# wild-firefox/FreeRL

Measured on AMD Instinct MI355X. Metric: learner_updates_per_sec, higher is better.
Workload: dtype f32; 1 GPU; TD3.learn() (BASELINE configs[1] algorithm; north_star synthetic shape): obs_dim 8, act_dim 2, batch 256, replay 1e6 rows filled, hidden 128, policy_freq 2, device-drawn indices/noise; learners_per_gpu=512, kernel_family=chained (one eight-wave workgroup per learner, two waves per SIMD), rows_per_workgroup=256, lds_bytes=160128, parallelism=seeds sharded over 1 GPU(s), no data-path collective, collective=metric all-reduce: none (single process)

## Files before the change

freerl_amd/csrc/device/chain_net.hpp:

```cpp
#pragma once
#include "chain.hpp"
#include "ppo_timing.hpp"

#if defined(FRL_PPO_TIMING) && defined(FRL_BWD_TIMING)
#define BWD_T0() long long b_prev_ = clock64()
#define BWD_T(i) do { const long long n_ = clock64(); if (threadIdx.x == 0 && blockIdx.x == 0) atomicAdd((unsigned long long*)&g_ppo_clk[1][i], (unsigned long long)(n_ - b_prev_)); b_prev_ = n_; } while (0)
#else
#define BWD_T0() do {} while (0)
#define BWD_T(i) do {} while (0)
#endif
#ifndef FRL_LANES_OPAQUE4
#define FRL_LANES_OPAQUE4 1
#endif
#ifndef FRL_FW_HALF
#define FRL_FW_HALF 1
#endif

namespace frl {

constexpr int kChainBatch = 256;


struct ChainLds {
    lds_f w1, w2, w3, b1, b2, b3, ls, ea, eb, ab, yb, q1, lpn, red, ex;
};
constexpr int chain_lds_floats() { return 8 * 256 + 64 * 256 + 8 * 256 + 2 * 8192 + 128 + 128 + 16 + 16 + kChainBatch * 4 + 3 * kChainBatch + 64; }
constexpr int chain8_lds_floats() { return chain_lds_floats() + 1024; }

template <int NW>
struct HeadGradT {
    static constexpr int OT = kHT / NW;
    f32x4 g2[OT][kHT], g1[OT], g3[OT];
    float gb1[OT], gb2[OT], gb3;
};
using HeadGrad = HeadGradT<4>;

typedef int i32x4_t __attribute__((ext_vector_type(4)));
struct AdamBuf { __amdgpu_buffer_rsrc_t th, mm, vv, tg; };
constexpr int kAdamDrop = 0x40000000;
__device__ __forceinline__ AdamBuf adam_buf(g_f th, g_f mA, g_f vA, g_f tg, int bytes) {
    AdamBuf B;
// ... 17 lines not shown
    return __builtin_nontemporal_load(reinterpret_cast<const FRL_GLB f32x4*>(p));
#else
    return ld4(p);
#endif
}
__device__ __forceinline__ f32x4 buf_ld4(__amdgpu_buffer_rsrc_t r, int voff, int soff) {
    return __builtin_bit_cast(f32x4, __builtin_amdgcn_raw_buffer_load_b128(r, voff, soff, FRL_ADAM_AUX_LD));
}
__device__ __forceinline__ void buf_st4(__amdgpu_buffer_rsrc_t r, int voff, int const_off, const f32x4& v) {
    __builtin_amdgcn_raw_buffer_store_b128(__builtin_bit_cast(i32x4_t, v), r, voff + const_off, 0, FRL_ADAM_AUX_ST);
}



template <int NW>
struct ChainNetT {
    static_assert(NW == 4 || NW == 8, "4 or 8 waves per workgroup");
    static constexpr int OT = kHT / NW, kThreads = 64 * NW, kRows = 16 * NW;
    using Grad = HeadGradT<NW>;
    ChainLds S;
    int tid, l, w, i16, q, fslot, tslot;
    int lane2, lane1;

    __device__ __forceinline__ void init(float* smem) {
        lds_f p = (lds_f)smem;
        S.w1 = p; p += kHT * 256;
        S.w2 = p; p += kHT * kHT * 256;
        S.w3 = p; p += kHT * 256;
        S.ea = p; p += kHT * 4 * 256;
        S.eb = p; p += kHT * 4 * 256;
        S.b1 = p; p += kHid;
        S.b2 = p; p += kHid;
        S.b3 = p; p += 16;
        S.ls = p; p += 16;
        if constexpr (NW == 4) {
            S.ab = p; p += kChainBatch * 4;
            S.yb = p; p += kChainBatch;
            S.q1 = p; p += kChainBatch;
            S.lpn = p; p += kChainBatch;
            S.red = p; p += 64;
            S.ex = S.ab;
        } else {
            S.yb = p; p += kChainBatch;
            S.q1 = p; p += kChainBatch;
            S.lpn = p; p += kChainBatch;
            S.red = p; p += 64;
            S.ab = p; p += kChainBatch * 4;
            S.ex = S.ab;
        }
        init_lanes();
    }
    __device__ __forceinline__ void init_lanes() {
        tid = threadIdx.x; l = tid & 63; w = __builtin_amdgcn_readfirstlane(tid >> 6); i16 = l & 15; q = l >> 4;
        fslot = (q * 16 + (i16 ^ q)) << 2;
        tslot = (((i16 >> 2) * 16) << 2) + (i16 & 3);
        lane2 = 4 * (w * OT * kHT * 256 + fslot);
        lane1 = 4 * (w * OT * 256 + fslot);
    }

    struct LaneK { int i16, q, fslot, tslot; };
    __device__ __forceinline__ LaneK lanes() const {
        int L = l;
        if constexpr (NW == 8 || FRL_LANES_OPAQUE4) asm volatile("" : "+v"(L));
        LaneK K;
        K.i16 = L & 15; K.q = L >> 4;
        K.fslot = (K.q * 16 + (K.i16 ^ K.q)) << 2;
        K.tslot = (((K.i16 >> 2) * 16) << 2) + (K.i16 & 3);
        return K;
    }

    struct StageRegs { f32x4 t2[64 / NW], t1[8 / NW], t3[8 / NW]; float bb1, bb2, bb3, lsv; };
    __device__ __forceinline__ StageRegs stage_fetch(g_cf th, int head, int extra_n = 0) const {
        th += head * kHeadFloats;
        StageRegs R;
#pragma unroll
        for (int j = 0; j < 64 / NW; ++j) R.t2[j] = ld4_stage(th + kL2w + 4 * (tid + kThreads * j));
// ... 484 lines not shown
```

freerl_amd/csrc/engine_plan.hpp:

```cpp
#pragma once
#include <algorithm>
#include <cstdarg>
#include <cstddef>
#include <cstdio>
#include <cstring>
#include <string>
#include <utility>
#include <vector>

#include "../../include/freerl_hip.h"
#include "frl_desc.h"

namespace frl {

inline int pad16(int x) { return (x + 15) / 16 * 16; }
inline int pad32(int x) { return (x + 31) / 32 * 32; }

inline constexpr char kFrlLearn[] = "frl_learn";
struct AlgoTraits {
    const char* name;
    const char* learn;
    const char* act_hint;
    bool index_action;
    bool discrete_head;
// ... 33 lines not shown
constexpr int kLdsDqnFused = dqn2_lds_floats() * (int)sizeof(float);
constexpr int kLdsChain4 = critic2_lds_floats() * (int)sizeof(float), kLdsChain8 = critic8_lds_floats() * (int)sizeof(float);
constexpr int kLdsSolo = std::max(solo_lds_floats(), critic2_lds_floats()) * (int)sizeof(float);
constexpr int kLdsSolow = solow_lds_floats() * (int)sizeof(float);
constexpr int kLdsWide = wide_lds_floats() * (int)sizeof(float), kLdsWide16 = wide16_lds_floats_host() * (int)sizeof(float);
constexpr int kLdsMasac = 160 * 1024;
constexpr int kLdsAtt = 160 * 1024;

struct PlanLimits {
    int n_cus = 256;
    int lds_per_cu = 160 * 1024;
};
struct PlanKnobs {
    int assume_cus = 0;
    int rc = 0;
    int cps = 0;
    bool solow_narrow = false;
    int critic_v2 = -1;
    int solo = -1;
    int solo_maxp = 2 * kSoloMaxP;
    int solow = -1;
    bool solow_helpers = true;
    int chain_waves = 8;
};
inline bool knob_flag(int tri, bool dflt) { return tri < 0 ? dflt : tri != 0; }

struct EngineFacts {
    LearnFamily family = FAM_ROWCHUNK;
    int lds_bytes = 0;
    bool has_nets = false;
    int noisy_per_set = 0;
    size_t idx_count = 0, noise_count = 0;
    size_t alpha_count = 0, steps_count = 0;
    int solo_stride = 0;
    int solow_row_wgs = 0;
    int solow_wgs = 0;
    size_t act_wk_slot = 0;
    int chain_waves = 8;
    int n_cus = 256;
    int lds_per_cu = 160 * 1024;
};
struct EnginePlan : EngineFacts {
    EngineDesc h;
};

__attribute__((format(printf, 2, 3))) inline int plan_refuse(std::string* message, const char* fmt, ...) {
    char buf[512];
    va_list ap;
    va_start(ap, fmt);
    vsnprintf(buf, sizeof buf, fmt, ap);
    va_end(ap);
    if (message) *message = buf;
    return FRL_ERR_INVALID;
}

inline int build_net(NetDesc& N, const std::vector<std::pair<int, int>>& layers_in , int heads,
                     int hidden_act, int out_act, int extra_n, int n_shadow = 0) {
    memset(&N, 0, sizeof N);
    std::vector<std::pair<int, int>> layers = layers_in;
    for (int i = 0; i < n_shadow; ++i) layers.push_back(layers_in.back());
    N.n_layers = (int)layers.size();
// ... 164 lines not shown
}

inline int dqn_split_for(const EngineDesc& h, int batch, int pc, int split_knob) {
    const int nchunks = (batch + 63) / 64;
    int split = (pc <= 16) ? std::min(std::min(4, nchunks), h.S) : 1;
    if (split_knob >= 0) split = std::max(1, std::min(std::min(split_knob, nchunks), h.S));
    return split;
}

inline int family_lds_bytes(LearnFamily fam, int chain_waves) {
    switch (fam) {
        case FAM_DQN_FUSED: return kLdsDqnFused;
        case FAM_CHAINED: return chain_waves == 4 ? kLdsChain4 : kLdsChain8;
        case FAM_SOLO: return kLdsSolo;
        case FAM_SOLOW: return kLdsSolow;
        case FAM_WIDE: return kLdsWide;
        case FAM_WIDE16: return kLdsWide16;
        case FAM_ATT: return kLdsAtt;
        case FAM_MASAC: return kLdsMasac;
        case FAM_ROWCHUNK: break;
    }
    return 0;
}

struct LearnPath { bool chained; int bytes, rows; };
inline LearnPath learn_path(const EngineDesc& h, const EngineFacts& f, LearnFamily fam, int batch, int dqn_split) {
    int bytes = family_lds_bytes(fam, f.chain_waves), rows = batch;
    switch (fam) {
        case FAM_ROWCHUNK: case FAM_ATT: case FAM_MASAC: bytes = f.lds_bytes; rows = h.rc; break;
        case FAM_DQN_FUSED: rows = std::min(((batch + 63) / 64 + dqn_split - 1) / dqn_split * 64, batch); break;
        case FAM_SOLO: bytes = solo_lds_floats() * (int)sizeof(float); rows = 16 * (kSoloWG / h.solo); break;
        case FAM_SOLOW: rows = 16 * (h.solow / std::max(1, f.solow_row_wgs)); break;
        default: break;
    }
    return {fam != FAM_ROWCHUNK && fam != FAM_ATT && fam != FAM_MASAC, bytes, rows};
}

inline int check_create_args(const frl_config& c, const frl_config_ext* ext, std::string* message) {
    int state_dim = 0;
    if (ext) {
        if (ext->size != (int)sizeof(frl_config_ext)) return plan_refuse(message, "frl_config_ext.size %d != sizeof(frl_config_ext) %d", ext->size, (int)sizeof(frl_config_ext));
        if (ext->state_dim < 0) return plan_refuse(message, "frl_config_ext.state_dim %d must be >= 0", ext->state_dim);
        if (ext->state_rows != FRL_STATE_ROWS_POSITION && ext->state_rows != FRL_STATE_ROWS_SAMPLE)
            return plan_refuse(message, "frl_config_ext.state_rows %d (FRL_STATE_ROWS_POSITION or FRL_STATE_ROWS_SAMPLE)", ext->state_rows);
        state_dim = ext->state_dim;
    }
// ... 169 lines not shown
        off += h.net[i].size;
        const int nl = h.net[i].n_layers / h.net[i].heads;
        if (c.algo == FRL_ALGO_MADDPG_ATT && (i & 1)) {
            kin = std::max(kin, h.net[i].L[ATT_E].k_pad);
            continue;
        }
        for (int hd = 0; hd < h.net[i].heads; ++hd) {
            kin = std::max(kin, h.net[i].L[hd * nl].k_pad);
            outp = std::max(outp, h.net[i].L[hd * nl + nl - 1].n_pad);
        }
    }
    h.learner_stride = pad32(off);
    h.lds_kin_pad = kin;
    h.lds_out_pad = outp;
}

inline int plan_sizes(const frl_config& c, const PlanKnobs& knobs, EnginePlan& pl, std::string* message) {
    EngineDesc& h = pl.h;
    const RecordDesc& R = h.rec;
    const AlgoTraits& T = algo_traits(c.algo);
    const int H = h.hidden;
    pl.family = choose_engine_family(pl, knobs);
    pl.chain_waves = knobs.chain_waves == 4 ? 4 : 8;
    h.act_max = 1;
    for (int j = 0; j < c.n_agents; ++j) h.act_max = std::max(h.act_max, R.act_dim[j]);
    h.lds_hbufs = 1;
    for (int i = 0; i < h.n_nets; ++i)
        if (h.net[i].n_layers / std::max(1, h.net[i].heads) > 2) h.lds_hbufs = 2;
    h.lds_batch_pad = 128;
    h.lds_act_pad = (std::max(R.act_total, 1) + 3) / 4 * 4;
    if (h.c51_atoms) h.lds_act_pad = std::max(h.lds_act_pad, (std::max(h.c51_atoms, c.act_dim[0]) + 3) / 4 * 4);
    if (T.vector_reward) h.lds_act_pad = std::max(h.lds_act_pad, (h.reward_dim + 3) / 4 * 4);
    bool one_wg_per_net = false;
    bool whole_cu = false;
    int call_rows = h.batch_max;
    switch (c.algo) {
        case FRL_ALGO_PPO:
            if (c.discrete) h.lds_act_pad = std::max(h.lds_act_pad, pad16(c.act_dim[0]));
            if (c.actor_dist == 1) h.lds_act_pad = std::max(h.lds_act_pad, pad16(2 * c.act_dim[0]));
            one_wg_per_net = true;
            break;
        case FRL_ALGO_SAC_DISCRETE:
            h.lds_act_pad = std::max(h.lds_act_pad, (c.act_dim[0] + 3) / 4 * 4);
            break;
        case FRL_ALGO_GAIL:
            h.lds_act_pad = std::max(h.lds_act_pad, ((H + 31) / 32 + 3) / 4 * 4);
// ... 125 lines not shown
```

freerl_amd/csrc/frl_api.hip:

```cpp
#include <hip/hip_runtime.h>

#include <chrono>
#include <cmath>
#include <cstdarg>
#include <cstdio>
#include <cstdlib>
#include <cstring>
#include <string>
#include <vector>

#include "../../include/freerl_hip.h"
#include "frl_desc.h"
#include "engine_plan.hpp"
#include "host_mem.hpp"

#include "kernels.h"
#ifdef FRL_UNITY
#include "kernels_replay.hip"
#include "kernels_update.hip"
#include "kernels_dqn.hip"
#include "kernels_critic.hip"
#include "kernels_actor.hip"
#include "kernels_act.hip"
#include "kernels_ppo.hip"
// ... 217 lines not shown
    if (e->stream) hipStreamDestroy(e->stream);
    delete e;
    return FRL_OK;
}

static LearnKernels resolve_learn_kernels(LearnFamily fam, int chain_waves, const EngineDesc& h);
static hipError_t set_family_lds_attributes(LearnFamily fam);

extern "C" int frl_create(const frl_config* cfg, frl_engine** out) { return frl_create_ex(cfg, nullptr, out); }

static PlanKnobs create_knobs() {
    auto tri = [](const char* name) { return env_set(name) ? (int)env_flag(name, false) : -1; };
    PlanKnobs k;
    k.assume_cus = env_int("FRL_ASSUME_CUS", k.assume_cus);
    k.rc = env_int("FRL_RC", k.rc);
    k.cps = env_int("FRL_CPS", k.cps);
    k.solow_narrow = env_flag("FRL_SOLOW_NARROW", k.solow_narrow);
    k.critic_v2 = tri("FRL_CRITIC_V2");
    k.solo = tri("FRL_SOLO");
    k.solo_maxp = env_int("FRL_SOLO_MAXP", k.solo_maxp);
    k.solow = tri("FRL_SOLOW");
    k.solow_helpers = env_flag("FRL_SOLOW_HELPERS", k.solow_helpers);
    k.chain_waves = env_int("FRL_CHAIN_WAVES", k.chain_waves);
    return k;
}

extern "C" int frl_create_ex(const frl_config* cfg, const frl_config_ext* ext, frl_engine** out) {
    if (!cfg || !out) return fail(FRL_ERR_INVALID, "cfg/out is NULL");
    *out = nullptr;
    const frl_config& c = *cfg;
    std::string why;
    if (const int rc = check_create_args(c, ext, &why)) return fail(rc, "%s", why.c_str());
    int ndev = 0;
    if (hipGetDeviceCount(&ndev) != hipSuccess || ndev == 0)
        return fail(FRL_ERR_NO_DEVICE, "no HIP device visible: the engine has no CPU fallback");
    if (c.device_id < 0 || c.device_id >= ndev) return fail(FRL_ERR_INVALID, "device_id %d of %d", c.device_id, ndev);
    HIP_TRY(hipSetDevice(c.device_id));
    PlanLimits limits;
    hipDeviceProp_t prop;
    if (hipGetDeviceProperties(&prop, c.device_id) == hipSuccess) {
        limits.n_cus = std::max(1, prop.multiProcessorCount);
        limits.lds_per_cu = (int)std::max<size_t>(prop.maxSharedMemoryPerMultiProcessor, prop.sharedMemPerBlock);
    }
    EnginePlan plan;
    if (const int rc = plan_engine(c, ext, limits, create_knobs(), &plan, &why)) return fail(rc, "%s", why.c_str());

// ... 1010 lines not shown
```

freerl_amd/csrc/frl_api_learn.inc:

```

enum LearnKernelStage { LK_CRITIC, LK_CRITIC_NV, LK_ACTOR, LK_STEP };
struct LearnKernelRow {
    LearnFamily fam;
    int stage;
    int sub;
    int lds_bytes;
    KernelPtr k[2][2];
};
static const LearnKernelRow kLearnKernels[] = {
    {FAM_DQN_FUSED, LK_CRITIC, 0, kLdsDqnFused, {{dqn_fused_kernel, dqn_fused_kernel}, {dqn_fused_kernel, dqn_fused_kernel}}},
    {FAM_CHAINED, LK_CRITIC, 8, kLdsChain8, {{ac_critic_v2_single_kernel, ac_critic_v2_single_kernel}, {ac_critic_v2_twin_kernel, ac_critic_v2_twin_kernel}}},
    {FAM_CHAINED, LK_CRITIC_NV, 8, kLdsChain8, {{ac_critic_v2_single_nv_kernel, ac_critic_v2_single_nv_kernel}, {ac_critic_v2_twin_nv_kernel, ac_critic_v2_twin_nv_kernel}}},
    {FAM_CHAINED, LK_ACTOR, 8, kLdsChain8, {{ac_actor_v2_kernel, ac_actor_v2_kernel}, {ac_actor_v2_kernel, ac_actor_v2_kernel}}},
    {FAM_CHAINED, LK_CRITIC, 4, kLdsChain4, {{ac_critic_v2w4_single_kernel, ac_critic_v2w4_single_kernel}, {ac_critic_v2w4_twin_kernel, ac_critic_v2w4_twin_kernel}}},
    {FAM_CHAINED, LK_ACTOR, 4, kLdsChain4, {{ac_actor_v2w4_kernel, ac_actor_v2w4_kernel}, {ac_actor_v2w4_kernel, ac_actor_v2w4_kernel}}},
    {FAM_SOLO, LK_CRITIC, 16, kLdsSolo, {{solo_critic_single_kernel, solo_critic_single_kernel}, {solo_critic_twin_kernel, solo_critic_twin_kernel}}},
    {FAM_SOLO, LK_ACTOR, 16, kLdsSolo, {{solo_actor_kernel, solo_actor_kernel}, {solo_actor_kernel, solo_actor_kernel}}},
    {FAM_SOLO, LK_CRITIC, 8, kLdsSolo, {{solo_critic_single_w8_kernel, solo_critic_single_w8_kernel}, {solo_critic_twin_w8_kernel, solo_critic_twin_w8_kernel}}},
    {FAM_SOLO, LK_ACTOR, 8, kLdsSolo, {{solo_actor_w8_kernel, solo_actor_w8_kernel}, {solo_actor_w8_kernel, solo_actor_w8_kernel}}},
    {FAM_SOLOW, LK_CRITIC, 1, kLdsSolow, {{solow_critic_h1a1_kernel, solow_critic_h1a2_kernel}, {solow_critic_h2a1_kernel, solow_critic_h2a2_kernel}}},
    {FAM_SOLOW, LK_ACTOR, 1, kLdsSolow, {{solow_actor_a1_kernel, solow_actor_a2_kernel}, {solow_actor_a1_kernel, solow_actor_a2_kernel}}},
    {FAM_SOLOW, LK_STEP, 1, kLdsSolow, {{solow_step_h1a1_kernel, solow_step_h1a2_kernel}, {solow_step_h2a1_kernel, solow_step_h2a2_kernel}}},
    {FAM_SOLOW, LK_CRITIC, 2, kLdsSolow, {{solow_critic_ma_h1a1_kernel, solow_critic_ma_h1a2_kernel}, {solow_critic_ma_h2a1_kernel, solow_critic_ma_h2a2_kernel}}},
    {FAM_SOLOW, LK_ACTOR, 2, kLdsSolow, {{solow_actor_ma_a1_kernel, solow_actor_ma_a2_kernel}, {solow_actor_ma_a1_kernel, solow_actor_ma_a2_kernel}}},
// ... 109 lines not shown
    prof_begin(e, actor ? PK_GRAD_ACTOR : PK_GRAD_CRITIC);
    hipLaunchKernelGGL(k, grid_chunks, dim3(256), e->lds_bytes, s.st, e->d, a, ns);
    prof_end(e);
    AdamArgs ad{};
    ad.ns = ns; ad.batch = a.batch; ad.eps = a.adam_eps; ad.beta1 = a.beta1; ad.beta2 = a.beta2; ad.clip = a.clip_norm;
    ad.tau = a.tau; ad.alpha_lr = a.alpha_lr; ad.target_entropy = a.target_entropy; ad.p0 = s.p0; ad.G = h.Gmax;
    if (actor) {
        ad.which = 1; ad.lr = a.actor_lr; ad.wd = 0.f; ad.soft = maddpg ? 0 : 1; ad.sac_alpha = sac ? 1 : 0;
    } else {
        ad.which = 0; ad.lr = a.critic_lr; ad.wd = a.critic_wd;
        ad.soft = (h.algo == ALGO_DQN) ? 1 : ((!maddpg && a.do_actor) ? 1 : 0);
    }
    prof_begin(e, actor ? PK_ADAM_ACTOR : PK_ADAM_CRITIC);
    launch_adam(e, s.st, ad, s.units, grid_adam);
    prof_end(e);
}

static void launch_chained(frl_engine* e, const LearnStage& s, LearnArgs a) {
    const LearnKernels& K = e->kern;
    LearnKernel k = K.actor.k;
    if (s.stage == 0) {
        a.stagger = env_int("FRL_STAGGER", 0);
        a.stagger_groups = env_int("FRL_STAGGER_GROUPS", 4); a.stagger_wgs = e->n_cus;
        const RecordDesc& R = e->h.rec;
        const bool nv = R.nobs_off[0] % 4 == 0 && R.nobs_off[0] + 16 <= R.stride && R.rew_off % 2 == 0 && R.done_off == R.rew_off + 1 && !env_set("FRL_CRITIC2_NOVEC");
        k = (nv && K.critic_nv.k) ? K.critic_nv.k : K.critic.k;
    }
    prof_begin(e, s.stage == 0 ? PK_GRAD_CRITIC : PK_GRAD_ACTOR);
    hipLaunchKernelGGL(k, dim3(s.pc), dim3(K.block), (size_t)K.lds_bytes, s.st, e->d, a);
    prof_end(e);
}

static void launch_wide(frl_engine* e, const LearnStage& s, const LearnArgs& a) {
    const LearnKernels& K = e->kern;
    prof_begin(e, s.stage == 0 ? PK_GRAD_CRITIC : PK_GRAD_ACTOR);
    hipLaunchKernelGGL(s.stage == 0 ? K.critic.k : K.actor.k, dim3(s.units), dim3(K.block), (size_t)K.lds_bytes, s.st, e->d, a);
    prof_end(e);
}

static SoloArgs solo_args(frl_engine* e) {
    SoloArgs sa{e->d_solo_slab, e->d_solo_part, e->d_solo_bar, e->d_solo_err, e->solo_bar_base, e->solo_stride, nullptr, nullptr, 0ull};
    if (e->h.solow) { sa.tiles = e->h.solow; sa.bar2 = e->d_solow_bar2; sa.row_wgs = e->solow_row_wgs; sa.update_wgs = e->solow_wgs; }
    e->solo_bar_base += kSoloWG;
    return sa;
}

static bool predraw_slots(frl_engine* e, SoloArgs& sa, size_t slot_stride, bool read, bool may_write) {
    if (read) sa.pre_read = e->d_solo_pre + (size_t)(e->solo_pre_seq & 1) * slot_stride;
    if (may_write) {
        sa.pre_write = e->d_solo_pre + (size_t)((e->solo_pre_seq + 1) & 1) * slot_stride;
        sa.pre_counter = e->rng_counter;
    }
// ... 243 lines not shown
```

freerl_amd/csrc/frl_desc.h:

```cpp
#pragma once
#include <stdint.h>

namespace frl {

constexpr int kMaxLayers = 7;
constexpr int kMaxAgents = 8;
constexpr int kMaxNets = 2 * kMaxAgents;

enum Act : int { ACT_NONE = 0, ACT_RELU = 1, ACT_TANH = 2, ACT_LEAKY_RELU = 3 };
constexpr float kLeakySlope = 0.01f;
enum Algo : int { ALGO_DQN = 0, ALGO_DDPG = 1, ALGO_TD3 = 2, ALGO_SAC = 3, ALGO_MADDPG = 4, ALGO_PPO = 5, ALGO_SAC_DISCRETE = 6,
                  ALGO_REINFORCE = 7, ALGO_ENVELOPE_DQN = 8, ALGO_ENVELOPE_DDPG = 9, ALGO_GAIL = 10, ALGO_MAPPO = 11, ALGO_IPPO = 12, ALGO_HAPPO = 13,
                  ALGO_MADDPG_ATT = 14, ALGO_MASAC = 15 };

struct LayerDesc {
    int n, k;
    int n_pad, k_pad;
    int w_off, b_off;
};

struct NetDesc {
    int n_layers;
    int size;
    int n_params;
// ... 145 lines not shown
};

struct LearnArgs {
    int batch;
    int size;
    int device_rng;
    int do_actor;
    float gamma, tau;
    float actor_lr, critic_lr, alpha_lr;
    float adam_eps, beta1, beta2;
    float critic_wd;
    float clip_norm;
    float policy_noise, noise_clip, max_action, policy_noise_scale;
    int use_policy_noise;
    float target_entropy;
    unsigned long long rng_counter;
    int p0, p_count;
    int double_dqn;
    int use_isw;
    int dqn_split;
    int stagger;
    int stagger_groups;
    int stagger_wgs;
    int fuse_actor;
    int huber;
    float huber_delta;
    int agent;
};

}
```

freerl_amd/csrc/kernels_actor2.hip:

```cpp
#include <hip/hip_runtime.h>

#include "kernels.h"
#include "device/chain_net.hpp"
#include "device/ppo_timing.hpp"

namespace frl {

template <int NW, int TA>
__device__ __forceinline__ void ac_actor_v2_body(const EngineDesc& D, const LearnArgs& a, float* smem) {
    constexpr int kRC = 16 * NW, kRowsT = kRC * TA;
    constexpr int kNC = kChainBatch / kRC, kNCT = kChainBatch / kRowsT;
    static_assert(kNCT >= 1, "a chunk of passes A / B is at most the whole batch");
    const int p = a.p0 + blockIdx.x;
    const RecordDesc& R = D.rec;
    const NetDesc& NA = D.net[0];
    const NetDesc& NC = D.net[1];
    using Net = ChainNetT<NW>;
    Net C;
    C.init(smem);
    const ChainLds& S = C.S;
    const int tid = C.tid, l = C.l, w = C.w, i16 = C.i16, q = C.q;
    const int B = a.batch, O = R.obs_dim[0], A = R.act_dim[0];
    const size_t lbase = (size_t)p * D.learner_stride;
    g_f thA = as_global(D.theta + lbase + D.net_off[0]);
    g_f tgA = as_global(D.target + lbase + D.net_off[0]);
    g_f mA = as_global(D.m + lbase + D.net_off[0]);
    g_f vA = as_global(D.v + lbase + D.net_off[0]);
    g_cf thC = as_global(D.theta + lbase + D.net_off[1]);
    g_cf ring = as_global(D.replay + (size_t)p * D.capacity * R.stride);
    g_ci idx = as_global_i(D.idx + (size_t)p * D.batch_max);
    const float invB = 1.f / (float)B;
    const bool sac = (D.algo == ALGO_SAC);
    const float alpha = sac ? D.alpha[p * 4 + 3] : 0.f;
    const int am = D.act_max;
    g_cf noise1 = as_global(D.noise + ((size_t)p * D.noise_sets + 1) * D.batch_max * am);
    const int nq = sac ? NC.heads : 1;
    const float dqv = sac ? -0.5f * invB : -invB;
    const int nchunks = (B + kRC - 1) / kRC, nch2 = (B + kRowsT - 1) / kRowsT;
    lds_f dab = S.eb;

    int ridxT[kNC], ridx[kNC];
#pragma unroll
    for (int j4 = 0; j4 < kNC; ++j4) {
        const int rowT = (j4 / TA) * kRowsT + 16 * TA * w + (j4 % TA) * 16 + i16, row = j4 * kRC + 16 * w + i16;
        ridxT[j4] = rowT < B ? idx[rowT] : -1;
// ... 10 lines not shown
            for (int cc = 1; cc < kNCT; ++cc) ri = c2 == cc ? ridxT[TA * cc + t] : ri;
            if (ri >= 0) {
                g_cf rec = ring + (size_t)ri * R.stride;
#pragma unroll
                for (int e = 0; e < 4; ++e)
                    if (4 * q + e < O) X.x[t][e] = rec[R.obs_off[0] + 4 * q + e];
            }
        }
        return X;
    };
    auto load_obs = [&](int c) {
        f32x4 x = {0.f, 0.f, 0.f, 0.f};
        const int ri = pick(ridx, c);
        if (ri >= 0) {
            g_cf rec = ring + (size_t)ri * R.stride;
#pragma unroll
            for (int e = 0; e < 4; ++e)
                if (4 * q + e < O) x[e] = rec[R.obs_off[0] + 4 * q + e];
        }
        return x;
    };

    float lpsum = 0.f;
    PPO_T0();
    RowIn2 nxt2 = load_obs2(0);
    typename Net::StageRegs pend = C.stage_fetch((g_cf)thA, 0, NA.extra_n);
    C.stage_commit(pend);
    PPO_T(0);
    for (int c2 = 0; c2 < nch2; ++c2) {
        const RowIn2 cur = nxt2;
        nxt2 = load_obs2(c2 + 1 < nch2 ? c2 + 1 : 0);
        if (c2 + 1 == nch2) pend = C.stage_fetch(thC, 0);
        f32x4 z[TA], h1[TA][kHT], h2[TA][kHT];
        C.template forward_vh<TA>(cur.x, h1, h2, z, A);
#pragma unroll
        for (int t = 0; t < TA; ++t) {
            const int row = c2 * kRowsT + 16 * TA * w + 16 * t + i16;
            if (q == 0 && row < kChainBatch) {
                f32x4 an = {0.f, 0.f, 0.f, 0.f};
#pragma unroll
                for (int r = 0; r < 4; ++r) {
                    if (r < A && row < B) {
                        if (sac) {
                            an[r] = sac_sample(z[t][r], S.ls[r], noise1[(size_t)row * am + r], lpsum);
                        } else {
                            an[r] = tanhf(z[t][r]);
                        }
// ... 113 lines not shown
    lds_barrier();
    auto red_sum = [&](int base) {
        float v = S.red[base];
#pragma unroll
        for (int i = 1; i < NW; ++i) v += S.red[base + i];
        return v;
    };
    float g_extra = 0.f, ss_extra = 0.f;
    if (sac) {
#pragma unroll
        for (int r = 0; r < 4; ++r) {
            if (r < A) {
                const float raw = S.ls[r];
                const float gr = log_std_grad_open(raw) ? red_sum(24 + 8 * r) : 0.f;
                ss_extra += gr * gr;
                if (i16 == r) g_extra = gr;
            }
        }
    }
    const float total = sqrtf(red_sum(0) + ss_extra);
    const float qtot = red_sum(8);
    const float lptot = red_sum(16);
    const int t = __float_as_int(S.red[56]) + 1;
    const double bc1 = 1.0 - powi_d((double)a.beta1, t), bc2 = 1.0 - powi_d((double)a.beta2, t);
    AdamCoef co;
    co.coef = a.clip_norm > 0.f ? fminf(a.clip_norm / (total + 1e-6f), 1.f) : 1.f;
    co.step = (float)((double)a.actor_lr / bc1); co.inv_bc2s = 1.f / (float)sqrt(bc2);
    co.w1 = 1.f - a.beta1; co.w2 = 1.f - a.beta2; co.beta2 = a.beta2; co.eps = a.adam_eps; co.wd = 0.f;
    co.tk = 1.f - a.tau; co.tau = a.tau;
    PPO_T(5);
    C.template adam_head<true, 0, true>(g, thA, mA, vA, tgA, co, O, A, g_extra, sac ? NA.extra_n : 0);
    PPO_T(6);
    PPO_TDUMP();
    if (tid == 0) {
        steps[0] = t;
        float* st = D.stats + (size_t)p * ST_COUNT;
        st[ST_ACTOR_LOSS] = actor_loss_stat(sac, qtot, lptot, alpha, invB);
        st[ST_ACTOR_GNORM] = total;
        if (sac) sac_alpha_step(D.alpha + p * 4, st, steps, alpha, -lptot * invB, a.target_entropy, a.beta1, a.beta2, a.alpha_lr);
    }
}

#ifndef FRL_ACTOR8_TA
#define FRL_ACTOR8_TA 1
#endif
__global__ __launch_bounds__(512) void ac_actor_v2_kernel(const EngineDesc* __restrict__ Dp, LearnArgs a) {
    extern __shared__ __attribute__((aligned(16))) float smem[];
    ac_actor_v2_body<8, FRL_ACTOR8_TA>(*Dp, a, smem);
}
__global__ __launch_bounds__(256) void ac_actor_v2w4_kernel(const EngineDesc* __restrict__ Dp, LearnArgs a) {
    extern __shared__ __attribute__((aligned(16))) float smem[];
    ac_actor_v2_body<4, 2>(*Dp, a, smem);
}

}
```

freerl_amd/csrc/kernels_critic2.hip:

```cpp
#include <hip/hip_runtime.h>

#include "kernels.h"
#include "device/chain_net.hpp"
#include "device/ppo_timing.hpp"

#if defined(FRL_BWD_TIMING)
#undef PPO_UDUMP
#define PPO_UDUMP() do {} while (0)
#endif

namespace frl {

#ifndef FRL_CRITIC2_TT
#define FRL_CRITIC2_TT 2
#endif
#ifndef FRL_CRITIC2_AHEAD
#define FRL_CRITIC2_AHEAD 1
#endif
template <bool TWIN, int TT, int NW, bool NVEC>
__device__ __forceinline__ void ac_critic_v2_body(const EngineDesc& D, const LearnArgs& a, float* smem) {
    constexpr int kRC = 16 * NW;
    constexpr int kRowsT = kRC * TT;
    constexpr int kNC = kChainBatch / kRC;
    constexpr int kNCT = kChainBatch / kRowsT;
    static_assert(kNCT >= 1, "a target-pass chunk is at most the whole batch");
    constexpr int NH = TWIN ? 2 : 1;
    const int p = a.p0 + blockIdx.x;
    const RecordDesc& R = D.rec;
    const NetDesc& NA = D.net[0];
    const NetDesc& NC = D.net[1];
    using Net = ChainNetT<NW>;
    Net C;
    C.init(smem);
    const ChainLds& S = C.S;
    const int tid = C.tid, l = C.l, w = C.w, i16 = C.i16, q = C.q;
    const int B = a.batch, O = R.obs_dim[0], A = R.act_dim[0], am = D.act_max;
    const bool sac = (D.algo == ALGO_SAC);
    const size_t lbase = (size_t)p * D.learner_stride;
    g_cf tgA = as_global(D.target + lbase + D.net_off[0]);
    g_cf tgC = as_global(D.target + lbase + D.net_off[1]);
    g_f thC = as_global(D.theta + lbase + D.net_off[1]);
    g_f tgCw = as_global(D.target + lbase + D.net_off[1]);
    g_f mC = as_global(D.m + lbase + D.net_off[1]);
    g_f vC = as_global(D.v + lbase + D.net_off[1]);
    g_cf ring = as_global(D.replay + (size_t)p * D.capacity * R.stride);
    g_ci idx = as_global_i(D.idx + (size_t)p * D.batch_max);
    g_cf noise0 = as_global(D.noise + (size_t)p * D.noise_sets * D.batch_max * am);
    const float alpha = sac ? D.alpha[p * 4 + 3] : 0.f;
    const float invB = 1.f / (float)B;
    const int nchunks = (B + kRC - 1) / kRC;

    int ridx[kNC];
#pragma unroll
    for (int c = 0; c < kNC; ++c) {
        const int row = c * kRC + 16 * w + i16;
        ridx[c] = idx[row < B ? row : B - 1];
    }
    const int xoff = R.obs_off[0] + 4 * q;
    struct RowIn { f32x4 x; };
    auto load_row = [&](int c) {
        RowIn X;
        X.x = ld4(ring + (size_t)pick(ridx, c) * R.stride + xoff);
        return X;
    };
    auto zero_pad = [&](const f32x4& x, int width) {
        f32x4 r;
#pragma unroll
        for (int e = 0; e < 4; ++e) r[e] = 4 * q + e < width ? x[e] : 0.f;
        return r;
    };
    int ridxT[kNC];
#pragma unroll
    for (int j4 = 0; j4 < kNC; ++j4) {
        const int row = (j4 / TT) * kRowsT + 16 * TT * w + (j4 % TT) * 16 + i16;
        ridxT[j4] = idx[row < B ? row : B - 1];
    }
    int colo[4];
#pragma unroll
    for (int e = 0; e < 4; ++e) colo[e] = R.nobs_off[0] + (NVEC ? 4 * q : (4 * q + e < O ? 4 * q + e : O - 1));
    struct RowIn2 { f32x4 x[TT]; float rew[TT], done[TT]; };
    auto tile_of = [&](const int (&v)[kNC], int c2, int t) {
        int r = v[t];
#pragma unroll
        for (int cc = 1; cc < kNCT; ++cc) r = c2 == cc ? v[TT * cc + t] : r;
        return r;
    };
    auto load_row2 = [&](bool want_rd, int c2) {
        RowIn2 X;
#pragma unroll
        for (int t = 0; t < TT; ++t) {
            g_cf rec = ring + (size_t)tile_of(ridxT, c2, t) * R.stride;
            if constexpr (NVEC) {
                typedef float f32x2 __attribute__((ext_vector_type(2)));
                X.x[t] = ld4(rec + colo[0]);
                const f32x2 rd = *reinterpret_cast<const FRL_GLB f32x2*>(rec + R.rew_off);
                X.rew[t] = rd[0]; X.done[t] = rd[1];
            } else {
#pragma unroll
                for (int e = 0; e < 4; ++e) X.x[t][e] = rec[colo[e]];
                X.rew[t] = rec[R.rew_off]; X.done[t] = rec[R.done_off];
            }
        }
        return X;
    };
    const int nch2 = (B + kRowsT - 1) / kRowsT;

    if (a.stagger > 0 && (int)blockIdx.x < a.stagger_wgs) {
        const int group = (blockIdx.x >> 3) & (a.stagger_groups - 1);
        for (int i = 0; i < group * a.stagger; ++i) __builtin_amdgcn_s_sleep(32);
    }
    PPO_T0();
    RowIn2 nxt2 = load_row2(false, 0);
    f32x4 nzr[kNC];
#pragma unroll
    for (int j4 = 0; j4 < kNC; ++j4) {
        nzr[j4] = f32x4{0.f, 0.f, 0.f, 0.f};
        const int row = (j4 / TT) * kRowsT + 16 * TT * w + (j4 % TT) * 16 + i16;
        if (q == 0 && row < B && (sac || a.use_policy_noise)) {
#pragma unroll
            for (int r = 0; r < 4; ++r)
                if (r < A) nzr[j4][r] = noise0[(size_t)row * am + r];
        }
    }
    typename Net::StageRegs pend = C.stage_fetch(tgA, 0, NA.extra_n);
    C.stage_commit(pend);
    PPO_T(0);
    PPO_U0();
    auto target_actor_chunk = [&](int c2, auto last_c) {
        constexpr bool last = decltype(last_c)::value;
        const RowIn2 cur = nxt2;
        nxt2 = load_row2(true, last ? 0 : c2 + 1);
        if constexpr (last && FRL_CRITIC2_AHEAD) pend = C.stage_fetch(tgC, 0);
        PPO_U(0);
        f32x4 xo[TT], z[TT], h1[TT][kHT], h2[TT][kHT];
#pragma unroll
        for (int t = 0; t < TT; ++t) xo[t] = zero_pad(cur.x[t], O);
        C.template forward_vh<TT>(xo, h1, h2, z, A);
        PPO_U(1);
        if constexpr (last && !FRL_CRITIC2_AHEAD) pend = C.stage_fetch(tgC, 0);
#pragma unroll
        for (int t = 0; t < TT; ++t) {
            const int row = c2 * kRowsT + 16 * TT * w + 16 * t + i16;
            const bool valid = row < B;
            if (q == 0 && row < kChainBatch) {
                f32x4 an = {0.f, 0.f, 0.f, 0.f};
                float lp = 0.f;
                f32x4 nr = nzr[t];
#pragma unroll
                for (int cc = 1; cc < kNCT; ++cc) nr = c2 == cc ? nzr[TT * cc + t] : nr;
                if (valid) {
                    if (sac) {
#pragma unroll
                        for (int r = 0; r < 4; ++r) {
                            if (r < A) an[r] = sac_sample(z[t][r], S.ls[r], nr[r], lp);
                        }
                    } else {
#pragma unroll
                        for (int r = 0; r < 4; ++r) {
                            if (r < A) {
                                float v = tanhf(z[t][r]);
                                if (a.use_policy_noise) v = td3_smooth(a, v, nr[r]);
                                an[r] = v;
                            }
                        }
                    }
                }
                st4(S.ab + row * 4, an);
                S.lpn[row] = lp;
            }
        }
        PPO_U(2);
    };
    for (int c2 = 0; c2 + 1 < nch2; ++c2) target_actor_chunk(c2, IC<0>{});
    target_actor_chunk(nch2 - 1, IC<1>{});
    PPO_T(1);
    RowIn nxt;
#pragma unroll
    for (int hd = 0; hd < NH; ++hd) {
        PPO_UR();
        C.stage_commit(pend);
        PPO_U(3);
        auto target_critic_chunk = [&](int c2, auto last_c) {
            constexpr bool last = decltype(last_c)::value;
            const RowIn2 cur = nxt2;
            if constexpr (!last) nxt2 = load_row2(true, c2 + 1);
            else if (hd + 1 < NH) nxt2 = load_row2(true, 0);
            else nxt = load_row(0);
            if constexpr (last && FRL_CRITIC2_AHEAD) pend = hd + 1 < NH ? C.stage_fetch(tgC, hd + 1) : C.stage_fetch((g_cf)thC, 0);
            f32x4 xb[TT], z[TT], h1[TT][kHT], h2[TT][kHT];
#pragma unroll
            for (int t = 0; t < TT; ++t) {
                const int row = c2 * kRowsT + 16 * TT * w + 16 * t + i16;
                xb[t] = zero_pad(cur.x[t], O);
#pragma unroll
                for (int e = 0; e < 4; ++e) {
                    const int f = 4 * q + e;
                    if (row < B && f >= O && f < O + A) xb[t][e] = S.ab[row * 4 + f - O];
                }
            }
            PPO_U(4);
            C.template forward_vh<TT>(xb, h1, h2, z, 1);
            PPO_U(5);
            if constexpr (last && !FRL_CRITIC2_AHEAD) pend = hd + 1 < NH ? C.stage_fetch(tgC, hd + 1) : C.stage_fetch((g_cf)thC, 0);
#pragma unroll
            for (int t = 0; t < TT; ++t) {
                const int row = c2 * kRowsT + 16 * TT * w + 16 * t + i16;
                if (q == 0 && row < B) {
                    float qv = z[t][0];
                    if (hd == 1) qv = fminf(S.q1[row], qv);
                    if (hd == NH - 1) {
                        const float rew = cur.rew[t], done = cur.done[t];
                        S.yb[row] = sac ? td_target_sac(rew, done, a.gamma, qv, alpha, S.lpn[row]) : td_target(rew, done, a.gamma, qv);
                    } else {
                        S.q1[row] = qv;
                    }
                }
            }
            PPO_U(6);
        };
        for (int c2 = 0; c2 + 1 < nch2; ++c2) target_critic_chunk(c2, IC<0>{});
        target_critic_chunk(nch2 - 1, IC<1>{});
    }
    PPO_UDUMP();
    PPO_T(2);
    typename Net::Grad G[NH];
    float lossp = 0.f;
#pragma unroll
    for (int hd = 0; hd < NH; ++hd) {
        typename Net::Grad& g = G[hd];
        C.grad_zero(g);
        PPO_T(3);
        C.stage_commit(pend);
        PPO_T(0);
        auto critic_chunk = [&](int c, auto last_c) {
            constexpr bool last = decltype(last_c)::value;
            const int row = c * kRC + 16 * w + i16;
            const bool valid = row < B;
            const RowIn cur = nxt;
            nxt = load_row(last ? 0 : c + 1);
            if constexpr (last && NW == 4) {
                if (hd + 1 < NH) pend = C.stage_fetch((g_cf)thC, hd + 1);
            }
            f32x4 xb[1] = {zero_pad(cur.x, O + A)}, z[1], h1[1][kHT], h2[1][kHT];
            PPO_T(4);
            C.template forward_vh<1>(xb, h1, h2, z, 1);
            PPO_T(5);
            f32x4 dz = {0.f, 0.f, 0.f, 0.f};
            if (q == 0 && valid) {
                float lrow, grow;
                td_loss_row(a, z[0][0] - S.yb[row], lrow, grow);
                dz[0] = grow * invB;
                lossp += lrow;
            }
            C.backward(g, xb[0], h1[0], h2[0], dz, 1, [&]() {
                if constexpr (last && NW == 8) {
                    if (hd + 1 < NH) pend = C.stage_fetch((g_cf)thC, hd + 1);
                }
            });
            PPO_T(6);
        };
        for (int c = 0; c + 1 < nchunks; ++c) critic_chunk(c, IC<0>{});
        critic_chunk(nchunks - 1, IC<1>{});
        C.grad_finish(g);
    }

    PPO_T(3);
    float ss = 0.f;
#pragma unroll
    for (int hd = 0; hd < NH; ++hd) ss += C.grad_sumsq(G[hd]);
    ss = wave_sum(ss);
    const float lsum = wave_sum(lossp);
    lds_barrier();
    int* steps = D.steps + (size_t)p * (kMaxNets + 1);
    if (l == 0) { S.red[w] = ss; S.red[8 + w] = lsum; }
    if (tid == 0) S.red[16] = __int_as_float(steps[1]);
    lds_barrier();
    float tot2 = S.red[0], loss = S.red[8];
#pragma unroll
    for (int i = 1; i < NW; ++i) { tot2 += S.red[i]; loss += S.red[8 + i]; }
    const float total = sqrtf(tot2);
    const int t = __float_as_int(S.red[16]) + 1;
    const AdamCoef co = adam_coef(total, a.clip_norm, t, a.critic_lr, a.beta1, a.beta2, a.adam_eps, a.critic_wd, a.tau);
#if !(FRL_ABL & 1)
    if (a.do_actor != 0) {
        static_for<0, NH>([&](auto hd) { C.template adam_head<true, decltype(hd)::value, decltype(hd)::value == NH - 1>(G[decltype(hd)::value], thC, mC, vC, tgCw, co, O + A, 1); });
    } else {
        static_for<0, NH>([&](auto hd) { C.template adam_head<false, decltype(hd)::value, decltype(hd)::value == NH - 1>(G[decltype(hd)::value], thC, mC, vC, tgCw, co, O + A, 1); });
    }
#else
    if (co.coef == 123.f) static_for<0, NH>([&](auto hd) { S.red[40 + decltype(hd)::value] = C.grad_sumsq(G[decltype(hd)::value]) * co.step; });
#endif
    PPO_T(7);
    PPO_TDUMP();
    if (tid == 0) {
        steps[1] = t;
        float* st = D.stats + (size_t)p * ST_COUNT;
        st[ST_CRITIC_LOSS] = loss * invB;
        st[ST_CRITIC_GNORM] = total;
    }
}

#ifndef FRL_CRITIC8_TT
#define FRL_CRITIC8_TT 1
#endif
#define FRL_CRITIC2_KERNEL(name, threads, twin, tt, nw, nvec)                                              \
    __global__ __launch_bounds__(threads) void name(const EngineDesc* __restrict__ Dp, LearnArgs a) {       \
        extern __shared__ __attribute__((aligned(16))) float smem[];                                       \
        ac_critic_v2_body<twin, tt, nw, nvec>(*Dp, a, smem);                                               \
    }
FRL_CRITIC2_KERNEL(ac_critic_v2_twin_kernel, 512, true, FRL_CRITIC8_TT, 8, false)
FRL_CRITIC2_KERNEL(ac_critic_v2_single_kernel, 512, false, FRL_CRITIC8_TT, 8, false)
FRL_CRITIC2_KERNEL(ac_critic_v2_twin_nv_kernel, 512, true, FRL_CRITIC8_TT, 8, true)
FRL_CRITIC2_KERNEL(ac_critic_v2_single_nv_kernel, 512, false, FRL_CRITIC8_TT, 8, true)
FRL_CRITIC2_KERNEL(ac_critic_v2w4_twin_kernel, 256, true, FRL_CRITIC2_TT, 4, false)
FRL_CRITIC2_KERNEL(ac_critic_v2w4_single_kernel, 256, false, FRL_CRITIC2_TT, 4, false)

}
```

Baseline: 827,400 updates/s.

## Make chained kernels persistent over learners and skew target/critic phases across learners

The eight-wave chained critic and actor kernels now launch at most one workgroup per CU and loop over learners with a grid stride, rather than launching one workgroup per learner. In the critic kernel, the target pass for a later learner can run ahead of the critic update of the current one, using alternating LDS target buffers. Prefetches of the next learner's critic weights and replay rows are issued across that boundary. Per-learner Adam scalars are pinned in scalar registers via an opaque asm. This aims to remove launch/tail imbalance and hide weight-fetch latency, but adds loop and register overhead and serializes learners within each workgroup.

```diff
diff --git a/freerl_amd/csrc/device/chain_net.hpp b/freerl_amd/csrc/device/chain_net.hpp
--- a/freerl_amd/csrc/device/chain_net.hpp
+++ b/freerl_amd/csrc/device/chain_net.hpp
@@ -17,6 +17,11 @@
 #endif
 
 namespace frl {
+
+__device__ __forceinline__ float per_learner(float x) {
+    asm volatile("" : "+s"(x));
+    return x;
+}
 
 constexpr int kChainBatch = 256;
 
@@ -80,7 +85,8 @@
     int tid, l, w, i16, q, fslot, tslot;
     int lane2, lane1;
 
-    __device__ __forceinline__ void init(float* smem) {
+    __device__ __forceinline__ void init(float* smem) { carve(smem); init_lanes(); }
+    __device__ __forceinline__ void carve(float* smem) {
         lds_f p = (lds_f)smem;
         S.w1 = p; p += kHT * 256;
         S.w2 = p; p += kHT * kHT * 256;
@@ -106,10 +112,10 @@
             S.ab = p; p += kChainBatch * 4;
             S.ex = S.ab;
         }
-        init_lanes();
-    }
-    __device__ __forceinline__ void init_lanes() {
-        tid = threadIdx.x; l = tid & 63; w = __builtin_amdgcn_readfirstlane(tid >> 6); i16 = l & 15; q = l >> 4;
+    }
+    __device__ __forceinline__ void init_lanes() { init_lanes((int)threadIdx.x); }
+    __device__ __forceinline__ void init_lanes(int t) {
+        tid = t; l = tid & 63; w = __builtin_amdgcn_readfirstlane(tid >> 6); i16 = l & 15; q = l >> 4;
         fslot = (q * 16 + (i16 ^ q)) << 2;
         tslot = (((i16 >> 2) * 16) << 2) + (i16 & 3);
         lane2 = 4 * (w * OT * kHT * 256 + fslot);
diff --git a/freerl_amd/csrc/engine_plan.hpp b/freerl_amd/csrc/engine_plan.hpp
--- a/freerl_amd/csrc/engine_plan.hpp
+++ b/freerl_amd/csrc/engine_plan.hpp
@@ -79,6 +79,7 @@
     int solow = -1;
     bool solow_helpers = true;
     int chain_waves = 8;
+    int chain_skew = 1;
 };
 inline bool knob_flag(int tri, bool dflt) { return tri < 0 ? dflt : tri != 0; }
 
@@ -94,6 +95,7 @@
     int solow_wgs = 0;
     size_t act_wk_slot = 0;
     int chain_waves = 8;
+    int chain_skew = 1;
     int n_cus = 256;
     int lds_per_cu = 160 * 1024;
 };
@@ -304,6 +306,8 @@
     }
     return 0;
 }
+
+inline int chained_grid(int p_count, int n_cus, int chain_waves) { return chain_waves == 4 ? p_count : std::min(p_count, std::max(1, n_cus)); }
 
 struct LearnPath { bool chained; int bytes, rows; };
 inline LearnPath learn_path(const EngineDesc& h, const EngineFacts& f, LearnFamily fam, int batch, int dqn_split) {
@@ -519,6 +523,7 @@
     const int H = h.hidden;
     pl.family = choose_engine_family(pl, knobs);
     pl.chain_waves = knobs.chain_waves == 4 ? 4 : 8;
+    pl.chain_skew = knobs.chain_skew == 0 || knobs.chain_skew == 2 ? knobs.chain_skew : 1;
     h.act_max = 1;
     for (int j = 0; j < c.n_agents; ++j) h.act_max = std::max(h.act_max, R.act_dim[j]);
     h.lds_hbufs = 1;
diff --git a/freerl_amd/csrc/frl_api.hip b/freerl_amd/csrc/frl_api.hip
--- a/freerl_amd/csrc/frl_api.hip
+++ b/freerl_amd/csrc/frl_api.hip
@@ -263,6 +263,7 @@
     k.solow = tri("FRL_SOLOW");
     k.solow_helpers = env_flag("FRL_SOLOW_HELPERS", k.solow_helpers);
     k.chain_waves = env_int("FRL_CHAIN_WAVES", k.chain_waves);
+    k.chain_skew = env_int("FRL_CHAIN_SKEW", k.chain_skew);
     return k;
 }
 
diff --git a/freerl_amd/csrc/frl_api_learn.inc b/freerl_amd/csrc/frl_api_learn.inc
--- a/freerl_amd/csrc/frl_api_learn.inc
+++ b/freerl_amd/csrc/frl_api_learn.inc
@@ -155,12 +155,13 @@
     if (s.stage == 0) {
         a.stagger = env_int("FRL_STAGGER", 0);
         a.stagger_groups = env_int("FRL_STAGGER_GROUPS", 4); a.stagger_wgs = e->n_cus;
+        a.chain_skew = e->chain_skew;
         const RecordDesc& R = e->h.rec;
         const bool nv = R.nobs_off[0] % 4 == 0 && R.nobs_off[0] + 16 <= R.stride && R.rew_off % 2 == 0 && R.done_off == R.rew_off + 1 && !env_set("FRL_CRITIC2_NOVEC");
         k = (nv && K.critic_nv.k) ? K.critic_nv.k : K.critic.k;
     }
     prof_begin(e, s.stage == 0 ? PK_GRAD_CRITIC : PK_GRAD_ACTOR);
-    hipLaunchKernelGGL(k, dim3(s.pc), dim3(K.block), (size_t)K.lds_bytes, s.st, e->d, a);
+    hipLaunchKernelGGL(k, dim3(chained_grid(s.pc, e->n_cus, e->chain_waves)), dim3(K.block), (size_t)K.lds_bytes, s.st, e->d, a);
     prof_end(e);
 }
 
diff --git a/freerl_amd/csrc/frl_desc.h b/freerl_amd/csrc/frl_desc.h
--- a/freerl_amd/csrc/frl_desc.h
+++ b/freerl_amd/csrc/frl_desc.h
@@ -191,6 +191,7 @@
     int stagger;
     int stagger_groups;
     int stagger_wgs;
+    int chain_skew;
     int fuse_actor;
     int huber;
     float huber_delta;
diff --git a/freerl_amd/csrc/kernels_actor2.hip b/freerl_amd/csrc/kernels_actor2.hip
--- a/freerl_amd/csrc/kernels_actor2.hip
+++ b/freerl_amd/csrc/kernels_actor2.hip
@@ -11,16 +11,21 @@
     constexpr int kRC = 16 * NW, kRowsT = kRC * TA;
     constexpr int kNC = kChainBatch / kRC, kNCT = kChainBatch / kRowsT;
     static_assert(kNCT >= 1, "a chunk of passes A / B is at most the whole batch");
-    const int p = a.p0 + blockIdx.x;
     const RecordDesc& R = D.rec;
     const NetDesc& NA = D.net[0];
     const NetDesc& NC = D.net[1];
     using Net = ChainNetT<NW>;
     Net C;
-    C.init(smem);
+    C.carve(smem);
     const ChainLds& S = C.S;
+    const int B = a.batch, O = R.obs_dim[0], A = R.act_dim[0];
+    PPO_T0();
+    const int p_end = NW == 8 ? a.p0 + a.p_count : a.p0 + (int)blockIdx.x + 1;
+    for (int p = a.p0 + (int)blockIdx.x; p < p_end; p += gridDim.x) {
+    int tx = threadIdx.x;
+    if constexpr (NW == 8) asm volatile("" : "+v"(tx));
+    C.init_lanes(tx);
     const int tid = C.tid, l = C.l, w = C.w, i16 = C.i16, q = C.q;
-    const int B = a.batch, O = R.obs_dim[0], A = R.act_dim[0];
     const size_t lbase = (size_t)p * D.learner_stride;
     g_f thA = as_global(D.theta + lbase + D.net_off[0]);
     g_f tgA = as_global(D.target + lbase + D.net_off[0]);
@@ -77,7 +82,6 @@
     };
 
     float lpsum = 0.f;
-    PPO_T0();
     RowIn2 nxt2 = load_obs2(0);
     typename Net::StageRegs pend = C.stage_fetch((g_cf)thA, 0, NA.extra_n);
     C.stage_commit(pend);
@@ -237,11 +241,12 @@
     const float qtot = red_sum(8);
     const float lptot = red_sum(16);
     const int t = __float_as_int(S.red[56]) + 1;
-    const double bc1 = 1.0 - powi_d((double)a.beta1, t), bc2 = 1.0 - powi_d((double)a.beta2, t);
+    const float lr_a = NW == 8 ? per_learner(a.actor_lr) : a.actor_lr, beta1 = NW == 8 ? per_learner(a.beta1) : a.beta1, beta2 = NW == 8 ? per_learner(a.beta2) : a.beta2;
+    const double bc1 = 1.0 - powi_d((double)beta1, t), bc2 = 1.0 - powi_d((double)beta2, t);
     AdamCoef co;
     co.coef = a.clip_norm > 0.f ? fminf(a.clip_norm / (total + 1e-6f), 1.f) : 1.f;
-    co.step = (float)((double)a.actor_lr / bc1); co.inv_bc2s = 1.f / (float)sqrt(bc2);
-    co.w1 = 1.f - a.beta1; co.w2 = 1.f - a.beta2; co.beta2 = a.beta2; co.eps = a.adam_eps; co.wd = 0.f;
+    co.step = (float)((double)lr_a / bc1); co.inv_bc2s = 1.f / (float)sqrt(bc2);
+    co.w1 = 1.f - beta1; co.w2 = 1.f - beta2; co.beta2 = beta2; co.eps = a.adam_eps; co.wd = 0.f;
     co.tk = 1.f - a.tau; co.tau = a.tau;
     PPO_T(5);
     C.template adam_head<true, 0, true>(g, thA, mA, vA, tgA, co, O, A, g_extra, sac ? NA.extra_n : 0);
@@ -252,7 +257,9 @@
         float* st = D.stats + (size_t)p * ST_COUNT;
         st[ST_ACTOR_LOSS] = actor_loss_stat(sac, qtot, lptot, alpha, invB);
         st[ST_ACTOR_GNORM] = total;
-        if (sac) sac_alpha_step(D.alpha + p * 4, st, steps, alpha, -lptot * invB, a.target_entropy, a.beta1, a.beta2, a.alpha_lr);
+        if (sac) sac_alpha_step(D.alpha + p * 4, st, steps, alpha, -lptot * invB, a.target_entropy, beta1, beta2, NW == 8 ? per_learner(a.alpha_lr) : a.alpha_lr);
+    }
+    if constexpr (NW == 4) break;
     }
 }
 
diff --git a/freerl_amd/csrc/kernels_critic2.hip b/freerl_amd/csrc/kernels_critic2.hip
--- a/freerl_amd/csrc/kernels_critic2.hip
+++ b/freerl_amd/csrc/kernels_critic2.hip
@@ -25,40 +25,33 @@
     constexpr int kNCT = kChainBatch / kRowsT;
     static_assert(kNCT >= 1, "a target-pass chunk is at most the whole batch");
     constexpr int NH = TWIN ? 2 : 1;
-    const int p = a.p0 + blockIdx.x;
     const RecordDesc& R = D.rec;
     const NetDesc& NA = D.net[0];
     const NetDesc& NC = D.net[1];
     using Net = ChainNetT<NW>;
     Net C;
-    C.init(smem);
+    C.carve(smem);
     const ChainLds& S = C.S;
-    const int tid = C.tid, l = C.l, w = C.w, i16 = C.i16, q = C.q;
+    int tid, l, w, i16, q, xoff, colo[4];
     const int B = a.batch, O = R.obs_dim[0], A = R.act_dim[0], am = D.act_max;
     const bool sac = (D.algo == ALGO_SAC);
-    const size_t lbase = (size_t)p * D.learner_stride;
-    g_cf tgA = as_global(D.target + lbase + D.net_off[0]);
-    g_cf tgC = as_global(D.target + lbase + D.net_off[1]);
-    g_f thC = as_global(D.theta + lbase + D.net_off[1]);
-    g_f tgCw = as_global(D.target + lbase + D.net_off[1]);
-    g_f mC = as_global(D.m + lbase + D.net_off[1]);
-    g_f vC = as_global(D.v + lbase + D.net_off[1]);
-    g_cf ring = as_global(D.replay + (size_t)p * D.capacity * R.stride);
-    g_ci idx = as_global_i(D.idx + (size_t)p * D.batch_max);
-    g_cf noise0 = as_global(D.noise + (size_t)p * D.noise_sets * D.batch_max * am);
-    const float alpha = sac ? D.alpha[p * 4 + 3] : 0.f;
     const float invB = 1.f / (float)B;
     const int nchunks = (B + kRC - 1) / kRC;
+    const int pstep = gridDim.x;
+    const int pfirst = a.p0 + (int)blockIdx.x;
+    const int kwalk = NW == 8 ? (a.p_count - (int)blockIdx.x + pstep - 1) / pstep : 1;
+    const int ahead = NW == 8 ? (a.chain_skew == 2 ? 1 : a.chain_skew == 1 ? (int)((blockIdx.x >> 3) & 1) : 0) : 0;
 
     int ridx[kNC];
-#pragma unroll
-    for (int c = 0; c < kNC; ++c) {
-        const int row = c * kRC + 16 * w + i16;
-        ridx[c] = idx[row < B ? row : B - 1];
-    }
-    const int xoff = R.obs_off[0] + 4 * q;
+    auto load_ridx = [&](g_ci idx) {
+#pragma unroll
+        for (int c = 0; c < kNC; ++c) {
+            const int row = c * kRC + 16 * w + i16;
+            ridx[c] = idx[row < B ? row : B - 1];
+        }
+    };
     struct RowIn { f32x4 x; };
-    auto load_row = [&](int c) {
+    auto load_row = [&](g_cf ring, int c) {
         RowIn X;
         X.x = ld4(ring + (size_t)pick(ridx, c) * R.stride + xoff);
         return X;
@@ -70,14 +63,22 @@
         return r;
     };
     int ridxT[kNC];
-#pragma unroll
-    for (int j4 = 0; j4 < kNC; ++j4) {
-        const int row = (j4 / TT) * kRowsT + 16 * TT * w + (j4 % TT) * 16 + i16;
-        ridxT[j4] = idx[row < B ? row : B - 1];
-    }
-    int colo[4];
-#pragma unroll
-    for (int e = 0; e < 4; ++e) colo[e] = R.nobs_off[0] + (NVEC ? 4 * q : (4 * q + e < O ? 4 * q + e : O - 1));
+    auto load_ridxT = [&](g_ci idx) {
+#pragma unroll
+        for (int j4 = 0; j4 < kNC; ++j4) {
+            const int row = (j4 / TT) * kRowsT + 16 * TT * w + (j4 % TT) * 16 + i16;
+            ridxT[j4] = idx[row < B ? row : B - 1];
+        }
+    };
+    auto relane = [&]() {
+        int tx = threadIdx.x;
+        if constexpr (NW == 8) asm volatile("" : "+v"(tx));
+        C.init_lanes(tx);
+        tid = C.tid; l = C.l; w = C.w; i16 = C.i16; q = C.q;
+        xoff = R.obs_off[0] + 4 * q;
+#pragma unroll
+        for (int e = 0; e < 4; ++e) colo[e] = R.nobs_off[0] + (NVEC ? 4 * q : (4 * q + e < O ? 4 * q + e : O - 1));
+    };
     struct RowIn2 { f32x4 x[TT]; float rew[TT], done[TT]; };
     auto tile_of = [&](const int (&v)[kNC], int c2, int t) {
         int r = v[t];
@@ -85,7 +86,7 @@
         for (int cc = 1; cc < kNCT; ++cc) r = c2 == cc ? v[TT * cc + t] : r;
         return r;
     };
-    auto load_row2 = [&](bool want_rd, int c2) {
+    auto load_row2 = [&](g_cf ring, bool want_rd, int c2) {
         RowIn2 X;
 #pragma unroll
         for (int t = 0; t < TT; ++t) {
@@ -110,7 +111,25 @@
         for (int i = 0; i < group * a.stagger; ++i) __builtin_amdgcn_s_sleep(32);
     }
     PPO_T0();
-    RowIn2 nxt2 = load_row2(false, 0);
+    PPO_U0();
+    typename Net::StageRegs pend;
+    RowIn nxt;
+    auto learner_ring = [&](int p) { return as_global(D.replay + (size_t)p * D.capacity * R.stride); };
+    auto learner_idx = [&](int p) { return as_global_i(D.idx + (size_t)p * D.batch_max); };
+    auto learner_theta_c = [&](int p) { return as_global(D.theta + (size_t)p * D.learner_stride + D.net_off[1]); };
+    auto target_phase = [&](const int p, lds_f yb, const int pc) {
+    relane();
+    const size_t lbase = (size_t)p * D.learner_stride;
+    g_cf tgA = as_global(D.target + lbase + D.net_off[0]);
+    g_cf tgC = as_global(D.target + lbase + D.net_off[1]);
+    g_cf thCn = learner_theta_c(pc);
+    g_cf ring = learner_ring(p), ringn = learner_ring(pc);
+    g_cf noise0 = as_global(D.noise + (size_t)p * D.noise_sets * D.batch_max * am);
+    const float alpha = sac ? D.alpha[p * 4 + 3] : 0.f;
+    lds_f q1 = yb;
+    load_ridx(learner_idx(pc));
+    load_ridxT(learner_idx(p));
+    RowIn2 nxt2 = load_row2(ring, false, 0);
     f32x4 nzr[kNC];
 #pragma unroll
     for (int j4 = 0; j4 < kNC; ++j4) {
@@ -122,14 +141,14 @@
                 if (r < A) nzr[j4][r] = noise0[(size_t)row * am + r];
         }
     }
-    typename Net::StageRegs pend = C.stage_fetch(tgA, 0, NA.extra_n);
+    pend = C.stage_fetch(tgA, 0, NA.extra_n);
     C.stage_commit(pend);
     PPO_T(0);
-    PPO_U0();
+    PPO_UR();
     auto target_actor_chunk = [&](int c2, auto last_c) {
         constexpr bool last = decltype(last_c)::value;
         const RowIn2 cur = nxt2;
-        nxt2 = load_row2(true, last ? 0 : c2 + 1);
+        nxt2 = load_row2(ring, true, last ? 0 : c2 + 1);
         if constexpr (last && FRL_CRITIC2_AHEAD) pend = C.stage_fetch(tgC, 0);
         PPO_U(0);
         f32x4 xo[TT], z[TT], h1[TT][kHT], h2[TT][kHT];
@@ -174,7 +193,6 @@
     for (int c2 = 0; c2 + 1 < nch2; ++c2) target_actor_chunk(c2, IC<0>{});
     target_actor_chunk(nch2 - 1, IC<1>{});
     PPO_T(1);
-    RowIn nxt;
 #pragma unroll
     for (int hd = 0; hd < NH; ++hd) {
         PPO_UR();
@@ -183,10 +201,10 @@
         auto target_critic_chunk = [&](int c2, auto last_c) {
             constexpr bool last = decltype(last_c)::value;
             const RowIn2 cur = nxt2;
-            if constexpr (!last) nxt2 = load_row2(true, c2 + 1);
-            else if (hd + 1 < NH) nxt2 = load_row2(true, 0);
-            else nxt = load_row(0);
-            if constexpr (last && FRL_CRITIC2_AHEAD) pend = hd + 1 < NH ? C.stage_fetch(tgC, hd + 1) : C.stage_fetch((g_cf)thC, 0);
+            if constexpr (!last) nxt2 = load_row2(ring, true, c2 + 1);
+            else if (hd + 1 < NH) nxt2 = load_row2(ring, true, 0);
+            else nxt = load_row(ringn, 0);
+            if constexpr (last && FRL_CRITIC2_AHEAD) pend = hd + 1 < NH ? C.stage_fetch(tgC, hd + 1) : C.stage_fetch(thCn, 0);
             f32x4 xb[TT], z[TT], h1[TT][kHT], h2[TT][kHT];
 #pragma unroll
             for (int t = 0; t < TT; ++t) {
@@ -201,18 +219,18 @@
             PPO_U(4);
             C.template forward_vh<TT>(xb, h1, h2, z, 1);
             PPO_U(5);
-            if constexpr (last && !FRL_CRITIC2_AHEAD) pend = hd + 1 < NH ? C.stage_fetch(tgC, hd + 1) : C.stage_fetch((g_cf)thC, 0);
+            if constexpr (last && !FRL_CRITIC2_AHEAD) pend = hd + 1 < NH ? C.stage_fetch(tgC, hd + 1) : C.stage_fetch(thCn, 0);
 #pragma unroll
             for (int t = 0; t < TT; ++t) {
                 const int row = c2 * kRowsT + 16 * TT * w + 16 * t + i16;
                 if (q == 0 && row < B) {
                     float qv = z[t][0];
-                    if (hd == 1) qv = fminf(S.q1[row], qv);
+                    if (hd == 1) qv = fminf(q1[row], qv);
                     if (hd == NH - 1) {
                         const float rew = cur.rew[t], done = cur.done[t];
-                        S.yb[row] = sac ? td_target_sac(rew, done, a.gamma, qv, alpha, S.lpn[row]) : td_target(rew, done, a.gamma, qv);
+                        yb[row] = sac ? td_target_sac(rew, done, a.gamma, qv, alpha, S.lpn[row]) : td_target(rew, done, a.gamma, qv);
                     } else {
-                        S.q1[row] = qv;
+                        q1[row] = qv;
                     }
                 }
             }
@@ -223,6 +241,15 @@
     }
     PPO_UDUMP();
     PPO_T(2);
+    };
+    auto critic_phase = [&](const int p, lds_cf yb) {
+    relane();
+    const size_t lbase = (size_t)p * D.learner_stride;
+    g_f thC = as_global(D.theta + lbase + D.net_off[1]);
+    g_f tgCw = as_global(D.target + lbase + D.net_off[1]);
+    g_f mC = as_global(D.m + lbase + D.net_off[1]);
+    g_f vC = as_global(D.v + lbase + D.net_off[1]);
+    g_cf ring = learner_ring(p);
     typename Net::Grad G[NH];
     float lossp = 0.f;
 #pragma unroll
@@ -237,7 +264,7 @@
             const int row = c * kRC + 16 * w + i16;
             const bool valid = row < B;
             const RowIn cur = nxt;
-            nxt = load_row(last ? 0 : c + 1);
+            nxt = load_row(ring, last ? 0 : c + 1);
             if constexpr (last && NW == 4) {
                 if (hd + 1 < NH) pend = C.stage_fetch((g_cf)thC, hd + 1);
             }
@@ -248,7 +275,7 @@
             f32x4 dz = {0.f, 0.f, 0.f, 0.f};
             if (q == 0 && valid) {
                 float lrow, grow;
-                td_loss_row(a, z[0][0] - S.yb[row], lrow, grow);
+                td_loss_row(a, z[0][0] - yb[row], lrow, grow);
                 dz[0] = grow * invB;
                 lossp += lrow;
             }
@@ -280,7 +307,8 @@
     for (int i = 1; i < NW; ++i) { tot2 += S.red[i]; loss += S.red[8 + i]; }
     const float total = sqrtf(tot2);
     const int t = __float_as_int(S.red[16]) + 1;
-    const AdamCoef co = adam_coef(total, a.clip_norm, t, a.critic_lr, a.beta1, a.beta2, a.adam_eps, a.critic_wd, a.tau);
+    const float lr_c = NW == 8 ? per_learner(a.critic_lr) : a.critic_lr, beta1 = NW == 8 ? per_learner(a.beta1) : a.beta1, beta2 = NW == 8 ? per_learner(a.beta2) : a.beta2;
+    const AdamCoef co = adam_coef(total, a.clip_norm, t, lr_c, beta1, beta2, a.adam_eps, a.critic_wd, a.tau);
 #if !(FRL_ABL & 1)
     if (a.do_actor != 0) {
         static_for<0, NH>([&](auto hd) { C.template adam_head<true, decltype(hd)::value, decltype(hd)::value == NH - 1>(G[decltype(hd)::value], thC, mC, vC, tgCw, co, O + A, 1); });
@@ -298,6 +326,24 @@
         st[ST_CRITIC_LOSS] = loss * invB;
         st[ST_CRITIC_GNORM] = total;
     }
+    };
+    auto cold_fetch = [&](const int p) {
+        relane();
+        load_ridx(learner_idx(p));
+        pend = C.stage_fetch(learner_theta_c(p), 0);
+        nxt = load_row(learner_ring(p), 0);
+    };
+    int t = 0;
+    for (int j = 0; j < kwalk; ++j) {
+        const int upto = j + ahead < kwalk - 1 ? j + ahead : kwalk - 1;
+        const int pc = pfirst + j * pstep;
+        if (t <= upto) {
+            do { target_phase(pfirst + t * pstep, (t & 1) ? S.q1 : S.yb, pc); ++t; } while (t <= upto);
+        } else {
+            cold_fetch(pc);
+        }
+        critic_phase(pc, (j & 1) ? S.q1 : S.yb);
+    }
 }
 
 #ifndef FRL_CRITIC8_TT
```

Result: no change. 830,300 updates/s (median of 6 runs) (+0.3%).
